# David-OConnor/molchanica

Hardware: AMD Instinct MI355X
Metric: MD atom-updates/sec (and steps/sec), 1M-atom solvated box (higher is better)
Workload: dtype f32

## Files before the change

molchanica_amd/csrc/mdx_api.hip:

```cpp
#include "mdx_comm.h"
#include <algorithm>
#include <atomic>
#include <chrono>
#include <cfloat>
#include <cmath>
#include <cstring>
#include <dlfcn.h>
#include <mutex>
#include <unordered_map>

static thread_local std::string g_last_error;
void mdx_set_error(const std::string& s) { g_last_error = s; }

static inline unsigned div_up(unsigned a, unsigned b) { return (a + b - 1) / b; }
static bool cut_on(float rc) { return rc > 0.f && std::isfinite(rc); }
static uint32_t f2u(float f) { uint32_t u; std::memcpy(&u, &f, 4); return u; }
static float u2f(uint32_t u) { float f; std::memcpy(&f, &u, 4); return f; }

#define FAIL(code, msg) do { mdx_set_error(msg); return (code); } while (0)

template <typename T>
static int upload_vec(T** dptr, const std::vector<T>& v, hipStream_t st) {
    if (*dptr) { (void)hipFree(*dptr); *dptr = nullptr; }
    HIP_TRY(hipMalloc((void**)dptr, std::max<size_t>(sizeof(T) * v.size(), 16)));
// ... 134 lines not shown
                    d.ps_cls, d.ps_p14, d.ps_stage, d.ps_slab, d.ps_rows, d.ps_fslab, d.ps_fout, d.ps_rigid, d.ps_flex, d.ps_flex_tab, d.ps_search, d.ps_cl, d.ps_cl_mat, d.gs_blk, d.gs_best, d.mx_blk};
    for (void* p : ptrs) if (p) (void)hipFree(p);
    d = DeviceState{};
}

extern "C" void mdx_destroy(mdx_handle* h) {
    if (!h) return;
    (void)hipSetDevice(h->device);
    if (h->stream) (void)hipStreamSynchronize(h->stream);
    mdx_dd_destroy(h);
    for (auto& e : h->ev_pending) { (void)hipEventDestroy(e.a); (void)hipEventDestroy(e.b); }
    for (auto& e : h->ev_pool) (void)hipEventDestroy(e);
    mdx_pme_destroy(h);
    free_device(h);
    if (h->h_ctl) (void)hipHostFree(h->h_ctl);
    if (h->h_rb) (void)hipHostFree(h->h_rb);
    if (h->stream) (void)hipStreamDestroy(h->stream);
    delete h;
}

static int create_impl(const mdx_system* s, const mdx_config* c, int device, mdx_handle* h) {
    const uint32_t N = s->n_atoms;
    h->N = N; h->cfg = *c; h->device = device;
    if (h->cfg.chunk_steps == 0) h->cfg.chunk_steps = N < 131072u ? 48u : 16u;
    if (h->cfg.chunk_steps > MDX_MAX_CHUNK) h->cfg.chunk_steps = MDX_MAX_CHUNK;
    decode_periodic(s->periodic, h->per);
    h->periodic = h->per[0] || h->per[1] || h->per[2];
    for (int d = 0; d < 3; ++d) h->posre_per[d] = h->per[d];
    for (int d = 0; d < 3; ++d) { h->box_lo[d] = s->box_lo[d]; h->box_hi[d] = s->box_hi[d]; }
    MDX_TRY(check_box(h->per, h->box_lo, h->box_hi, c));
    h->n_local = N; h->cap_local = N;
    const bool all_cut = cut_on(c->lj_cutoff) && cut_on(c->coulomb_cutoff);
    if (c->skin == 0.f && all_cut && h->periodic) {
        float s0 = 2.0f;
        for (int d = 0; d < 3; ++d)
            if (h->per[d]) s0 = std::min(s0, 0.5f * (h->box_hi[d] - h->box_lo[d]) - std::max(c->lj_cutoff, c->coulomb_cutoff) - 0.01f);
        if (s0 >= 0.5f) { h->cfg.skin = s0; h->skin_tune.on = true; h->skin_tune.base_skin = s0; MDX_TRY(check_box(h->per, h->box_lo, h->box_hi, &h->cfg)); }
    }
    h->r_list = all_cut ? std::max(c->lj_cutoff, c->coulomb_cutoff) + h->cfg.skin : INFINITY;

    int ndev = 0;
    if (hipGetDeviceCount(&ndev) != hipSuccess || ndev == 0) FAIL(MDX_EDEVICE, "no HIP device available");
    if (device < 0 || device >= ndev) FAIL(MDX_EDEVICE, "device index out of range");
    HIP_TRY(hipSetDevice(device));
    h->pme_cus_per_xcd = mdx_pme_cu_split(h, c);
    if (h->pme_cus_per_xcd) MDX_TRY(mdx_stream_create_masked(&h->stream, h->pme_cus_per_xcd, true));
    else HIP_TRY(hipStreamCreateWithFlags(&h->stream, hipStreamNonBlocking));
// ... 348 lines not shown
    if (h->profile_level == 2 && kind != 0 && kind != 4) return;
    if (h->profile_level == 2) {
        static const uint32_t every = [] { const char* e = std::getenv("MDX_PROF_SAMPLE"); const int v = e ? std::atoi(e) : 8; return (uint32_t)(v < 1 ? 1 : v); }();
        if (kind == 0) h->prof_sampled = (h->prof_seq++ % every) == 0u;
        if (!h->prof_sampled) return;
    }
    if (kind >= 6 && h->profile_level != 3) return;
    h->prof_open = true;
    mdx_handle::EvPair p{};
    p.kind = kind; p.tag = h->prof_tag; p.st = st ? st : h->stream;
    hipEvent_t* ev[2] = {&p.a, &p.b};
    for (auto e : ev) {
        if (!h->ev_pool.empty()) { *e = h->ev_pool.back(); h->ev_pool.pop_back(); }
        else (void)hipEventCreate(e);
    }
    (void)hipEventRecord(p.a, p.st);
    h->ev_pending.push_back(p);
}
void mdx_prof_end(mdx_handle* h) {
    if (!h->profile || !h->prof_open || h->ev_pending.empty()) return;
    h->prof_open = false;
    (void)hipEventRecord(h->ev_pending.back().b, h->ev_pending.back().st);
}
void mdx_prof_collect(mdx_handle* h, int first_stale_step) {
    for (auto& p : h->ev_pending) {
        float ms = 0.f;
        (void)hipEventSynchronize(p.b);
        const bool ran = p.tag < 0 || ((p.kind == 2 || p.kind == 5) ? p.tag <= first_stale_step : p.tag < first_stale_step);
        if (ran && hipEventElapsedTime(&ms, p.a, p.b) == hipSuccess) {
            if (p.kind == 0) { h->stats.nb_ms_sum += ms; h->stats.nb_launches++; }
            else if (p.kind == 4) h->stats.nb_ms_sum += ms;
            else if (p.kind == 1) { h->stats.bonded_ms_sum += ms; h->stats.bonded_launches++; }
            else if (p.kind == 2) { h->stats.integ_ms_sum += ms; h->stats.integ_launches++; }
            else if (p.kind == 5) { h->stats.fused_ms_sum += ms; h->stats.fused_launches++; }
            if (h->dd && h->profile_level == 3) {
                int ph = -1;
                if (p.kind >= 6 && p.kind <= 11) ph = p.kind - 6;
                else if (p.kind == 0) ph = MDX_PHASE_PAIR;
                else if (p.kind == 4) ph = MDX_PHASE_PAIR_BOUNDARY;
                else if (p.kind == 1 || p.kind == 5) ph = MDX_PHASE_BONDED;
                else if (p.kind == 2) ph = MDX_PHASE_INTEGRATE;
                if (ph >= 0) { h->dd->phase_ms[ph] += ms; h->dd->phase_n[ph]++; }
            }
        }
        h->ev_pool.push_back(p.a); h->ev_pool.push_back(p.b);
    }
    h->ev_pending.clear();
}

static void skin_apply(mdx_handle* h, float s) {
    h->cfg.skin = s;
    h->r_list = std::max(h->cfg.lj_cutoff, h->cfg.coulomb_cutoff) + s;
    h->list_valid = false;
    h->inner_skin_auto = 0.f; h->dual_auto_off = false; h->dual_win_steps = 0; h->dual_win_prunes = 0;
    h->stretch_samples = 0;
    h->skin_tune.win_steps = 0; h->skin_tune.win_rebuilds = 0; h->skin_tune.skip_rebuilds = 5;
}
static bool skin_fits(const mdx_handle* h, float s) {
    for (int d = 0; d < 3; ++d)
        if (h->per[d] && h->box_hi[d] - h->box_lo[d] < 2.0f * (std::max(h->cfg.lj_cutoff, h->cfg.coulomb_cutoff) + s)) return false;
    return true;
}
static void skin_autotune(mdx_handle* h, uint32_t done, bool stale_hit) {
    mdx_handle::SkinTune& t = h->skin_tune;
    const auto now = std::chrono::steady_clock::now();
    if (t.phase == 0) {
        t.warm_steps += done;
        if (t.warm_steps >= 200) { t.phase = 1; t.win_steps = 0; t.win_rebuilds = 0; t.skip_rebuilds = 1; }
        return;
    }
// ... 32 lines not shown
    const auto t0 = std::chrono::steady_clock::now();
    HIP_TRY(hipSetDevice(h->device));
    hipStream_t st = h->stream;
    DeviceState& d = h->d;
    const bool had_ext = h->have_ext;
    if (ext_forces) {
        if (h->n_local != h->N && !h->dd) FAIL(MDX_EPARAM, "external forces need the library's own decomposition (mdx_comm_init) on a narrowed handle");
        std::vector<float4> e4(h->N);
        for (uint32_t i = 0; i < h->N; ++i)
            e4[i] = make_float4(ext_forces[3 * i], ext_forces[3 * i + 1], ext_forces[3 * i + 2], 0.f);
        HIP_TRY(hipMemcpyAsync(d.ext_orig, e4.data(), sizeof(float4) * h->N, hipMemcpyHostToDevice, st));
        HIP_TRY(hipStreamSynchronize(st));
        h->have_ext = true; h->forces_valid = false;
    } else if (had_ext) {
        h->have_ext = false; h->forces_valid = false;
    }
    if (n_steps == 0) return MDX_OK;
    MDX_TRY(ensure_ready(h));
    if (h->moved_outside) { h->prune_pending = true; h->moved_outside = false; }
    uint32_t thr = stale_threshold_bits(h);
    uint32_t remaining = n_steps;
    while (remaining) {
        MDX_TRY(ensure_ready(h));
        uint32_t chunk = std::min(std::min(remaining, h->cfg.chunk_steps), mdx_steps_to_next_event(h));
        static const bool chunk_predict = [] { const char* e = std::getenv("MDX_CHUNK_PREDICT"); return !(e && e[0] == '0'); }();
        if (chunk_predict && h->stretch_samples >= 3 && chunk > 4) {
            const float left = h->stretch_mean + h->stretch_dev + 1.0f - (float)h->steps_since_rebuild;
            const uint32_t want = left > 4.0f ? (uint32_t)std::ceil(left) : 4u;
            chunk = std::min(chunk, want);
        }
        const auto t_chunk = std::chrono::steady_clock::now();
        MdxRange range_chunk("mdx step chunk");
        HIP_TRY(hipMemsetAsync(d.ctl, 0, sizeof(StepCtl), st));
        static const bool rattle_every = [] { const char* e = std::getenv("MDX_RATTLE_EVERY_STEP"); return e && e[0] == '1'; }();
        const int integ = h->integrator;
        const bool vv = integ == MDX_INTEGRATOR_VERLET_VELOCITY;
        const bool fused = vv && (!mdx_has_constraints(h) || !rattle_every);
        const bool fuse_bi = fused && mdx_bonded_integrate_ok(h);
        const bool want_e = mdx_energy_wanted_at(h, h->step_count + chunk);
        h->e_cache_valid = false; h->e_pending = false;
        const size_t e_bytes = sizeof(double) * (EN_COUNT + 8 + MDX_ESTRIDE * MDX_EPART);
        float4* pos_after[MDX_MAX_CHUNK + 1];
        const bool water = fused && mdx_water_step_ok(h);
        const bool pipe_chunk = fuse_bi && mdx_dd_fold_eligible(h);
        const bool onepass = fused && !water && !pipe_chunk && chunk >= (want_e ? 2u : 1u) && mdx_onepass_ok(h);
        float4* const ybuf[2] = {d.posq_alt, d.posq};
        float4* const fb3[3] = {d.force, d.force_b, d.force_c};
        auto onepass_point_at = [&](uint32_t n) {
// ... 71 lines not shown
        }
        h->prof_tag = -1;
        if (h->dd) { h->chunk_s = -1; mdx_dd_pipe_chunk_end(h); }
        static const bool dbg_host = [] { const char* e = std::getenv("MDX_DEBUG_HOST"); return e && e[0] == '1'; }();
        const auto t_enq = std::chrono::steady_clock::now();
        if (h->dd) h->dd->probe_both_buffers = fuse_bi && chunk > 1;
        MDX_TRY(ctl_to_host(h));
        if (h->dd) h->dd->probe_both_buffers = false;
        if (dbg_host && chunk >= 8) {
            static double enq = 0.0, wait = 0.0; static unsigned long long steps = 0, chunks = 0;
            const auto t_w = std::chrono::steady_clock::now();
            enq += std::chrono::duration<double, std::micro>(t_enq - t_chunk).count();
            wait += std::chrono::duration<double, std::micro>(t_w - t_enq).count();
            steps += chunk; ++chunks;
            if ((chunks & 31ull) == 0ull)
                std::fprintf(stderr, "[mdx host] %llu steps in %llu chunks: enqueue %.1f us per step, wait at the chunk end %.1f us per step\n",
                             steps, chunks, enq / (double)steps, wait / (double)steps);
        }
        uint32_t done = chunk;
        bool stale_hit = false;
        int first_stale = 1 << 30;
        for (uint32_t s = 0; s < chunk; ++s)
            if (h->h_ctl->disp2[s + 1] > thr || (onepass && h->h_ctl->viol[s])) { first_stale = (int)s; break; }
        if (h->profile) mdx_prof_collect(h, first_stale);
        static const bool dbg_stale = [] { const char* e = std::getenv("MDX_DEBUG_STALE"); return e && e[0] == '1'; }();
        if (dbg_stale && first_stale < (1 << 30))
            std::fprintf(stderr, "[mdx] list stale at step %d of a chunk of %u (step count %llu): word %.4g against (skin / 2)^2 = %.4g%s\n", first_stale, chunk,
                         (unsigned long long)h->step_count, (double)u2f(h->h_ctl->disp2[first_stale + 1]), (double)u2f(thr), h->dd ? " [decomposed]" : "");
        for (uint32_t s = 0; s < chunk; ++s) {
            const bool kick_beyond_grant = onepass && h->h_ctl->viol[s] != 0u;
            if (h->h_ctl->disp2[s + 1] > thr || kick_beyond_grant) {
                if (fuse_bi && !onepass && d.posq != pos_after[s]) std::swap(d.posq, d.posq_alt);
                if (onepass) {
                    onepass_point_at(s + 1);
                    MDX_TRY(mdx_launch_step_materialise(h, dt, ybuf[s & 1], fb3[s % 3], ybuf[(s + 1) & 1], kick_beyond_grant, s == 0 ? 0.5f : 1.0f, nullptr, 0));
                    if (kick_beyond_grant) ++h->onepass_violations;
                }
                if (u2f(h->h_ctl->disp2[s + 1]) > 1.0e29f) {
                    h->forces_valid = false; h->list_valid = false;
                    h->step_count += s;
                    FAIL(MDX_ENAN, "non-finite or runaway coordinates during mdx_step");
                }
                h->list_valid = false;
                const float len = (float)(h->steps_since_rebuild + s + 1);
                if (h->dd) { h->chunk_s = -1; MDX_TRY(mdx_dd_on_stale(h)); }
                else MDX_TRY(mdx_rebuild(h));
                {
                    if (h->stretch_samples == 0) { h->stretch_mean = len; h->stretch_dev = 2.0f; }
                    else {
                        h->stretch_dev += 0.25f * (std::fabs(len - h->stretch_mean) - h->stretch_dev);
                        h->stretch_mean += 0.25f * (len - h->stretch_mean);
                    }
                    ++h->stretch_samples;
                    stale_hit = true;
                }
                const bool e_now = want_e && s + 1 == chunk;
                if (e_now) HIP_TRY(hipMemsetAsync(d.energy, 0, e_bytes, st));
                h->nb_post_rebuild = !e_now;
                const int frc = compute_forces(h, e_now, nullptr, 0);
                h->nb_post_rebuild = false;
                MDX_TRY(frc);
                if (vv) {
                    MDX_TRY(mdx_launch_integrate(h, 2, dt, nullptr, nullptr, thr));
                    if (dt != 0.f) MDX_TRY(mdx_launch_constrain_velocities(h, nullptr, 0));
                }
                done = s + 1;
                break;
            }
        }
        if (h->dd) h->dd->spec_valid = false;
        if (h->dual_on && h->cfg.inner_skin == 0.f) {
            for (uint32_t s = 0; s < done; ++s) h->dual_win_prunes += h->h_ctl->prune[s + 1] != 0u;
            if (stale_hit && !h->inner_from_rebuild) ++h->dual_win_prunes;
            h->dual_win_steps += done;
            if (h->dual_win_steps >= 96) {
                const float f = (float)h->dual_win_prunes / (float)h->dual_win_steps;
                if (f > 0.30f) {
                    if (h->inner_skin + 0.25f <= h->cfg.skin - 0.75f) {
                        h->inner_skin_auto = h->inner_skin + 0.25f; h->inner_skin = h->inner_skin_auto;
                        h->prune_pending = true;
                    } else {
                        h->dual_auto_off = true; h->dual_on = false;
                    }
                }
                h->dual_win_steps = 0; h->dual_win_prunes = 0;
            }
        }
        if (h->dd && h->dd->world > 1 && h->dd->tune_phase < 2 && h->tile_split) {
            MdxDecomp* dd = h->dd;
            if (done == chunk && chunk == h->cfg.chunk_steps) {
                if (dd->tune_chunks >= 2) {
                    dd->tune_ms[dd->tune_phase] += std::chrono::duration<double, std::milli>(std::chrono::steady_clock::now() - t_chunk).count();
// ... 692 lines not shown
    if (n) hipLaunchKernelGGL(unpack_pos_kernel, dim3(div_up(n, 256)), dim3(256), 0, h->stream, n, d_gid,
                              h->d.slot_of, h->d.posq, (const float4*)d_in4, (const float4*)d_shift4,
                              flag_word >= 0 ? &h->d.ctl->disp2[flag_word] : nullptr,
                              dual ? h->d.ref : nullptr,
                              dual ? (mdx_dd_split_now(h) ? &h->d.ctl->prune_ghost[h->chunk_s + 1]
                                                                                                      : &h->d.ctl->prune[h->chunk_s + 1]) : nullptr,
                              0.5f * h->inner_skin * (1.0f - 1.0e-4f),
                              h->dd ? h->box_hi[0] - h->box_lo[0] : 0.f, h->dd ? h->box_hi[1] - h->box_lo[1] : 0.f,
                              h->dd ? h->box_hi[2] - h->box_lo[2] : 0.f, (dual && h->path_split) ? h->d.path : nullptr);
    HIP_TRY(hipGetLastError());
    h->forces_valid = false;
    if (!dual) h->moved_outside = true;
    return MDX_OK;
}

extern "C" void* mdx_stream(mdx_handle* h) { return h ? (void*)h->stream : nullptr; }
extern "C" int mdx_debug_half_stats(mdx_handle* h, unsigned long long out[6]) {
    HIP_TRY(hipStreamSynchronize(h->stream));
    HIP_TRY(hipMemcpy(out, h->d.inner_count + MDX_EPART, sizeof(unsigned long long) * 6, hipMemcpyDeviceToHost));
    return MDX_OK;
}

extern "C" int mdx_debug_pair_lists(mdx_handle* h, int which, uint32_t* dst, uint64_t capacity, uint64_t* n_out) {
    if (!h || !n_out || which < 0 || which > 5) FAIL(MDX_EPARAM, "bad argument");
    if (!h->in_slot_space || !h->d.list_counts || !h->d.entry_off) FAIL(MDX_EPARAM, "spatial caches not built");
    HIP_TRY(hipStreamSynchronize(h->stream));
    const DeviceState& d = h->d;
    const uint32_t T = h->T;
    const void* src = nullptr;
    uint64_t n = 0;
    if (which == 0) { src = d.list_counts; n = 2ull * T; }
    else if (which == 1) { src = d.entry_off; n = (uint64_t)T + 1; }
    else if (which == 4) { src = d.inner_nch; n = d.inner_nch ? 8ull * T : 0; }
    else if (which == 5) { src = d.orig_of; n = (uint64_t)T * MDX_TILE; }
    else {
        std::vector<ListCounts> cnt(T);
        std::vector<uint32_t> off((size_t)T + 1);
        if (T) HIP_TRY(hipMemcpy(cnt.data(), d.list_counts, sizeof(ListCounts) * T, hipMemcpyDeviceToHost));
        HIP_TRY(hipMemcpy(off.data(), d.entry_off, sizeof(uint32_t) * ((size_t)T + 1), hipMemcpyDeviceToHost));
        uint64_t ext = 0;
        for (uint32_t t = 0; t < T; ++t) ext = std::max<uint64_t>(ext, (uint64_t)off[t] + cnt[t].n_masked + cnt[t].n_plain);
        src = which == 2 ? d.entries : d.entries_in;
        n = src ? 2 * ext : 0;
    }
    *n_out = n;
    if (!dst) return MDX_OK;
    if (capacity < n) FAIL(MDX_EPARAM, "capacity below the number of words");
    if (n) HIP_TRY(hipMemcpy(dst, src, sizeof(uint32_t) * n, hipMemcpyDeviceToHost));
    return MDX_OK;
}

static int posre_install(mdx_handle* h) {
    DeviceState& d = h->d;
    hipStream_t st = h->stream;
    const uint32_t N = h->N, R_old = h->n_roles, n = h->n_posre;
    std::vector<uint32_t> off_old(N + 1);
    std::vector<RoleRec> rec_old(R_old);
// ... 104 lines not shown
```

molchanica_amd/csrc/mdx_grid.hip:

```cpp
#include "mdx_internal.h"
#include <atomic>
#include <chrono>
#include <algorithm>
#include <cfloat>
#include <cmath>

#define WAVE_LDS_SYNC()                                      \
    do {                                                     \
        __builtin_amdgcn_fence(__ATOMIC_SEQ_CST, "workgroup"); \
        __builtin_amdgcn_wave_barrier();                     \
    } while (0)

static inline unsigned div_up(unsigned a, unsigned b) { return (a + b - 1) / b; }

constexpr int SCAN_THREADS = 256;
constexpr int SCAN_ITEMS = 8;
constexpr int SCAN_TILE = SCAN_THREADS * SCAN_ITEMS;

template <int THREADS>
__device__ __forceinline__ uint32_t block_exclusive_scan(uint32_t v, uint32_t* s_wave , uint32_t* total) {
    const int lane = threadIdx.x & 63, wave = threadIdx.x >> 6;
    uint32_t inc = v;
#pragma unroll
    for (int d = 1; d < 64; d <<= 1) {
// ... 1290 lines not shown
    hipLaunchKernelGGL(readback_kernel, dim3(1), dim3(1), 0, h->stream, s, (volatile uint32_t*)h->h_rb, seq);
    if (h->profile) { HIP_TRY(hipStreamSynchronize(h->stream)); return MDX_OK; }
    return spin_on_readback(h, seq);
}

__global__ void cursor_sum_kernel(const unsigned long long* __restrict__ cursors, uint32_t* __restrict__ out) {
    const unsigned long long c = cursors[(size_t)threadIdx.x * 16];
    uint32_t e = (uint32_t)c, m = (uint32_t)(c >> 32);
#pragma unroll
    for (int k = 32; k > 0; k >>= 1) { e += __shfl_xor(e, k); m += __shfl_xor(m, k); }
    if (threadIdx.x == 0) { out[0] = e; out[1] = m; }
}

__global__ void pair_sum_kernel(unsigned long long* __restrict__ pc) {
    unsigned long long a = pc[(size_t)threadIdx.x * PC_STRIDE], b = pc[(size_t)threadIdx.x * PC_STRIDE + 1];
#pragma unroll
    for (int k = 32; k > 0; k >>= 1) { a += __shfl_xor(a, k); b += __shfl_xor(b, k); }
    if (threadIdx.x == 0) { pc[PC_TOTAL] = a; pc[PC_TOTAL + 1] = b; }
}

static float c_inner_skin(const mdx_config& c) { return c.inner_skin == 0.f ? 0.5f : c.inner_skin; }

constexpr uint32_t LPT_BUCKETS = 129;
enum { RB_T = 0, RB_T_OWN = 1, RB_NONFINITE = 2, RB_N_INT = 3, RB_SCAN_N = 4, RB_WORDS = 8 };

template <bool UNSORT>
__global__ __launch_bounds__(256) void rb_prep_kernel(uint32_t N, GridParams g, const uint32_t* __restrict__ gid, const uint32_t* __restrict__ slot_of,
                                                      const float4* __restrict__ posq, const float4* __restrict__ vel,
                                                      float4* __restrict__ pos_orig, float4* __restrict__ vel_orig,
                                                      const uint8_t* __restrict__ lflag, uint32_t* __restrict__ cell_of,
                                                      uint32_t* __restrict__ cell_k, uint32_t* __restrict__ cell_count,
                                                      uint32_t* __restrict__ nonfinite) {
    const uint32_t o = blockIdx.x * blockDim.x + threadIdx.x;
    if (o >= N) return;
    float4 p;
    if (UNSORT) { const uint32_t sl = slot_of[gid[o]]; p = posq[sl]; vel_orig[o] = vel[sl]; }
    else p = pos_orig[o];
    if (!(isfinite(p.x) && isfinite(p.y) && isfinite(p.z))) {
        *nonfinite = 1u;
        p.x = g.lo[0]; p.y = g.lo[1]; p.z = g.lo[2];
    }
    if (g.per[0]) p.x = wrap1(p.x, g.lo[0], g.len[0]);
    if (g.per[1]) p.y = wrap1(p.y, g.lo[1], g.len[1]);
    if (g.per[2]) p.z = wrap1(p.z, g.lo[2], g.len[2]);
    pos_orig[o] = p;
    const int cx = min(g.ncx - 1, max(0, mdx_col_of(g, 0, p.x)));
    const int cy = min(g.ncy - 1, max(0, mdx_col_of(g, 1, p.y)));
// ... 133 lines not shown
    }
    float lo[3] = {valid ? p.x : 3.0e38f, valid ? p.y : 3.0e38f, valid ? p.z : 3.0e38f};
    float hi[3] = {valid ? p.x : -3.0e38f, valid ? p.y : -3.0e38f, valid ? p.z : -3.0e38f};
#pragma unroll
    for (int m = 1; m < 8; m <<= 1)
#pragma unroll
        for (int d = 0; d < 3; ++d) { lo[d] = fminf(lo[d], __shfl_xor(lo[d], m)); hi[d] = fmaxf(hi[d], __shfl_xor(hi[d], m)); }
    const unsigned long long bv = __ballot(valid), bo = __ballot((fl & 2u) != 0);
    const unsigned long long kl = __ballot(l.y != 0.f), kq = __ballot(p.w != 0.f);
    if ((lane & 7) == 0) {
        const uint32_t c = t * MDX_CL_PER_TILE + (uint32_t)(lane >> 3);
        a.cl_lo[c] = make_float4(lo[0], lo[1], lo[2], (float)__popcll((bv >> lane) & 0xFFull));
        a.cl_hi[c] = make_float4(hi[0], hi[1], hi[2], (float)__popcll((bo >> lane) & 0xFFull));
        a.cl_kind[c] = (uint8_t)((((kl >> lane) & 0xFFull) ? 1u : 0u) | (((kq >> lane) & 0xFFull) ? 2u : 0u));
    }
}

struct LptSortLds { uint32_t hist[8 * LPT_BUCKETS], cur[8 * LPT_BUCKETS], scan[SCAN1_THREADS / 64]; };
__host__ __device__ inline uint32_t mdx_lpt_group_tiles(uint32_t T, uint32_t wpt) {
    const uint32_t tpb = (wpt > (uint32_t)MDX_NB_WAVES ? wpt : (uint32_t)MDX_NB_WAVES) / wpt;
    return (((T + tpb - 1u) / tpb + 7u) >> 3) * tpb;
}
__device__ __forceinline__ uint32_t lpt_counting_sort(uint32_t T, const ListCounts* __restrict__ counts, uint32_t group_tiles,
                                                      const uint32_t* __restrict__ is_int, uint32_t* __restrict__ order, LptSortLds& s) {
    constexpr uint32_t NB = 8 * LPT_BUCKETS;
    for (uint32_t b = threadIdx.x; b < NB; b += SCAN1_THREADS) s.hist[b] = 0;
    __syncthreads();
    auto bucket = [&](uint32_t t) {
        const uint32_t nch = (counts[t].n_masked + counts[t].n_plain) >> 3;
        const uint32_t major = group_tiles ? min(t / group_tiles, 7u) : ((is_int && !is_int[t]) ? 1u : 0u);
        return major * LPT_BUCKETS + LPT_BUCKETS - 1u - min(nch, LPT_BUCKETS - 1u);
    };
    for (uint32_t t = threadIdx.x; t < T; t += SCAN1_THREADS) atomicAdd(&s.hist[bucket(t)], 1u);
    __syncthreads();
    {
        const uint32_t b0 = 2u * threadIdx.x, h0 = b0 < NB ? s.hist[b0] : 0u, h1 = b0 + 1u < NB ? s.hist[b0 + 1u] : 0u;
        uint32_t tot;
        const uint32_t ex = block_exclusive_scan<SCAN1_THREADS>(h0 + h1, s.scan, &tot);
        if (b0 < NB) s.cur[b0] = ex;
        if (b0 + 1u < NB) s.cur[b0 + 1u] = ex + h0;
    }
    __syncthreads();
    const uint32_t n_major0 = s.cur[LPT_BUCKETS];
    __syncthreads();
    for (uint32_t t = threadIdx.x; t < T; t += SCAN1_THREADS) order[atomicAdd(&s.cur[bucket(t)], 1u)] = t;
    __syncthreads();
    return n_major0;
}

struct FinishArgs {
    uint32_t* rb_ctl; const ListCounts* counts;
    uint32_t* tile_lpt; uint32_t lpt_grouped; WptRule rule;
    const uint32_t* tile_int; uint32_t* tile_order;
    const unsigned long long* cursors; unsigned long long* pair_count; const uint32_t* flags;
    volatile uint32_t* host; uint32_t seq;
};
__global__ __launch_bounds__(SCAN1_THREADS) void rb_finish_kernel(FinishArgs a) {
    __shared__ LptSortLds s_sort;
    __shared__ uint32_t s_nint;
    const uint32_t T = a.rb_ctl[RB_T];
    if (threadIdx.x == 0) s_nint = 0u;
    if (a.tile_lpt) {
        const uint32_t group_tiles = a.lpt_grouped ? mdx_lpt_group_tiles(T, (uint32_t)mdx_wpt_rule(a.rule, T)) : 0u;
        (void)lpt_counting_sort(T, a.counts, group_tiles, nullptr, a.tile_lpt, s_sort);
    }
    if (a.tile_order) {
        const uint32_t n_int = lpt_counting_sort(T, a.counts, 0u, a.tile_int, a.tile_order, s_sort);
        if (threadIdx.x == 0) s_nint = n_int;
    }
    if (threadIdx.x < 64) {
        const unsigned long long c = a.cursors[(size_t)threadIdx.x * 16];
        uint32_t e = (uint32_t)c, m = (uint32_t)(c >> 32);
        unsigned long long pa = a.pair_count[(size_t)threadIdx.x * PC_STRIDE], pb = a.pair_count[(size_t)threadIdx.x * PC_STRIDE + 1];
#pragma unroll
        for (int k = 32; k > 0; k >>= 1) { e += __shfl_xor(e, k); m += __shfl_xor(m, k); pa += __shfl_xor(pa, k); pb += __shfl_xor(pb, k); }
        if (threadIdx.x == 0) {
            a.pair_count[PC_TOTAL] = pa; a.pair_count[PC_TOTAL + 1] = pb;
            a.rb_ctl[RB_N_INT] = s_nint;
            a.host[0] = T; a.host[1] = a.rb_ctl[RB_T_OWN]; a.host[2] = a.rb_ctl[RB_NONFINITE]; a.host[3] = s_nint;
            for (int k = 0; k < 4; ++k) a.host[4 + k] = a.flags[k];
            a.host[8] = e; a.host[9] = m;
            a.host[10] = (uint32_t)pa; a.host[11] = (uint32_t)(pa >> 32); a.host[12] = (uint32_t)pb; a.host[13] = (uint32_t)(pb >> 32);
            a.rb_ctl[RB_NONFINITE] = 0u;
            __threadfence_system();
            a.host[31] = a.seq;
        }
    }
}


struct RebuildKnobs {
    bool fused;
    bool two_pass;
    bool exact_prune;
    int inner_mode;
    uint32_t mw_below;
    bool list_debug;
    bool prune_hitbits;
    int prune_tries[2];
};
constexpr int PRUNE_HB_TRIES[2] = {1, 1};
constexpr uint32_t PRUNE_MW_BELOW_FUSED = 12000u, PRUNE_MW_BELOW_UNFUSED = 2048u;
static const RebuildKnobs& rebuild_knobs() {
    static const RebuildKnobs k = [] {
        auto env = [](const char* name) { const char* e = std::getenv(name); return e ? e : ""; };
        RebuildKnobs r;
        r.fused = env("MDX_REBUILD_FUSED")[0] != '0';
        r.two_pass = env("MDX_LIST_TWO_PASS")[0] == '1';
        r.exact_prune = env("MDX_EXACT_PRUNE")[0] != '0';
        const char in = env("MDX_REBUILD_INNER")[0];
        r.inner_mode = in == '0' ? 0 : (in == '2' ? 2 : 1);
        const char* const mw = std::getenv("MDX_PRUNE_MW_BELOW");
        r.mw_below = mw ? (uint32_t)std::atoi(mw) : PRUNE_MW_BELOW_FUSED;
        r.list_debug = std::getenv("MDX_LIST_DEBUG") != nullptr;
        r.prune_hitbits = env("MDX_PRUNE_HITBITS")[0] != '0';
        const char* const tr[2] = {std::getenv("MDX_PRUNE_TRIES"), std::getenv("MDX_PRUNE_TRIES_INNER")};
        for (int k = 0; k < 2; ++k) r.prune_tries[k] = tr[k] ? std::min(std::max(std::atoi(tr[k]), 0), 3) : PRUNE_HB_TRIES[k];
        return r;
    }();
    return k;
}

struct RebuildResult { uint32_t E = 0, MC = 0; unsigned long long npairs = 0; bool ordered = false, classified = false, inner_built = false; };

struct TileOrderPlan { bool lpt, grouped, split; };
static TileOrderPlan tile_order_plan(const mdx_handle* h, uint32_t T) {
    static const int lpt_env = [] { const char* e = std::getenv("MDX_TILE_LPT"); return e ? (e[0] == '0' ? 0 : (e[0] == '2' ? 2 : 1)) : -1; }();
    const bool decomposed = h->dd || h->n_local != h->N;
    TileOrderPlan p;
    p.lpt = (lpt_env >= 0 ? lpt_env >= 1 : (decomposed || T >= 512u)) && mdx_nb_variant(h) >= 2;
    p.grouped = lpt_env >= 0 ? lpt_env == 2 : !decomposed;
    p.split = h->want_tile_split && mdx_nb_variant(h) >= 2;
    return p;
}

static bool list_is_pruned(const mdx_handle* h) { return !std::isinf(h->r_list) && mdx_nb_variant(h) >= 2; }

static float next_inner_skin(const mdx_handle* h) { return h->inner_skin_auto > 0.f ? h->inner_skin_auto : c_inner_skin(h->cfg); }
static bool dual_list_wanted(const mdx_handle* h, float inner_skin) {
    return !h->dual_auto_off && mdx_nb_half(h) && list_is_pruned(h) && inner_skin > 0.f && inner_skin < h->cfg.skin &&
// ... 147 lines not shown
    ListArgs a = list_args(h, T_bound, d.rb_ctl + RB_T);
    launch_single_pass(h, &a);
    const bool inner_env = knobs.inner_mode == 2 || (knobs.inner_mode == 1 && !mdx_has_constraints(h) && h->n_vsites == 0);
    const float inner_skin_next = next_inner_skin(h);
    const bool inner_here = inner_env && prune && dual_list_wanted(h, inner_skin_next) && !h->dd && h->n_local == h->N && g.npop == 1 && !h->alch_on &&
                            d.entries_in && d.inner_nch;
    PruneInner pin{};
    if (inner_here) {
        pin.entries_in = d.entries_in; pin.inner_nch = d.inner_nch; pin.rule = mdx_wpt_rule_of(h);
        const float rin = std::max(std::isfinite(h->cfg.lj_cutoff) && h->cfg.lj_cutoff > 0.f ? h->cfg.lj_cutoff : 0.f,
                                   std::isfinite(h->cfg.coulomb_cutoff) && h->cfg.coulomb_cutoff > 0.f ? h->cfg.coulomb_cutoff : 0.f) + inner_skin_next;
        pin.rin2 = rin * rin;
    }
    const bool inner_launched = prune && launch_exact_prune(h, a, knobs.mw_below, d.rb_ctl, classify_here ? d.tile_bnd : nullptr, inner_here ? &pin : nullptr);
    MDX_TRY(mdx_remap_constraints(h));
    const uint32_t seq = ++h->rb_seq;
    {
        FinishArgs fa{};
        fa.rb_ctl = d.rb_ctl; fa.counts = d.list_counts;
        fa.tile_lpt = plan.lpt ? d.tile_lpt : nullptr; fa.lpt_grouped = plan.grouped ? 1u : 0u; fa.rule = mdx_wpt_rule_of(h);
        fa.tile_int = classify_here ? d.tile_bnd : nullptr; fa.tile_order = classify_here ? d.tile_order : nullptr;
        fa.cursors = reinterpret_cast<const unsigned long long*>(d.list_cursors); fa.pair_count = d.pair_count; fa.flags = d.flags_dev;
        fa.host = (volatile uint32_t*)h->h_rb; fa.seq = seq;
        hipLaunchKernelGGL(rb_finish_kernel, dim3(1), dim3(SCAN1_THREADS), 0, st, fa);
    }
    HIP_TRY(hipGetLastError());
    MDX_TRY(spin_on_readback(h, seq));
    const uint32_t T = h->h_rb[0], flags0 = h->h_rb[4];
    if (h->h_rb[2]) { h->cell_count_clean = false; mdx_set_error("non-finite position at neighbour rebuild"); return MDX_ENAN; }
    if (T > T_bound) { mdx_set_error("internal: tile count beyond its bound"); return MDX_EDEVICE; }
    h->T = T; h->S = (T + 1) * MDX_TILE;
    MDX_TRY(list_flags_error(flags0 & 1u));
    if (flags0 & (16u | 32u)) {
        if (knobs.list_debug) fprintf(stderr, "[mdx] fused list rebuild fell back: flags %u, T %u, cap_e %llu cap_m %u regions %u\n",
                                      flags0, T, (unsigned long long)h->cap_entries, h->cap_mchunks, a.n_regions);
        *fell_back = true;
        return MDX_OK;
    }
    MDX_TRY(list_flags_error(flags0));
    res->E = h->h_rb[8]; res->MC = h->h_rb[9];
    const unsigned long long built = (unsigned long long)h->h_rb[10] | ((unsigned long long)h->h_rb[11] << 32);
    const unsigned long long kept = (unsigned long long)h->h_rb[12] | ((unsigned long long)h->h_rb[13] << 32);
    res->npairs = prune ? kept : built;
    res->ordered = true;
    res->inner_built = inner_launched && mdx_wpt_rule(mdx_wpt_rule_of(h), T) == 1;
    h->force_zeroed = true;
    h->tile_lpt_on = plan.lpt; h->tile_lpt_grouped = plan.grouped;
// ... 155 lines not shown
        h->tile_split = false; h->n_interior = 0;
        if (plan.split) MDX_TRY(mdx_classify_tiles(h, plan.lpt));
    }
    if (!res.ordered) {
        h->tile_lpt_on = false;
        if (plan.lpt) MDX_TRY(mdx_order_tiles_by_length(h, plan.grouped));
    }
    h->list_valid = true;
    h->forces_valid = false;
    h->rebuild_count++; h->steps_since_rebuild = 0;
    mdx_dd_note_rebuild(h);
    h->inner_skin = next_inner_skin(h);
    h->dual_on = dual_list_wanted(h, h->inner_skin);
    h->prune_pending = !(res.inner_built && h->dual_on);
    h->inner_from_rebuild = !h->prune_pending;
    if (h->inner_from_rebuild) ++h->inner_rebuilds;
    h->tail_w = 0; h->tail_tiles = 0;
    if (h->dual_on && h->tile_lpt_on && h->tile_lpt_grouped && !h->alch_on) mdx_tail_plan(h, T, &h->tail_w, &h->tail_tiles);
    if (!d.inner_count) { ALLOC(d.inner_count, MDX_EPART + 8); HIP_TRY(hipMemsetAsync(d.inner_count, 0, sizeof(unsigned long long) * (MDX_EPART + 8), st)); }
    h->stats.n_atoms = h->n_local; h->stats.n_slots = S; h->stats.n_tiles = T; h->stats.n_clusters = NC;
    h->stats.n_list_entries = res.E; h->stats.n_masked_entries = (uint64_t)res.MC * 8;
    h->stats.n_cluster_pairs = (mdx_nb_variant(h) >= 2) ? res.npairs : (uint64_t)res.E * 8;
    if (h->profile) {
        float ms = 0.f;
        HIP_TRY(hipEventRecord(e1, st)); HIP_TRY(hipEventSynchronize(e1));
        HIP_TRY(hipEventElapsedTime(&ms, e0, e1));
        h->stats.rebuild_ms_sum += ms;
        h->ev_pool.push_back(e0); h->ev_pool.push_back(e1);
    }
    return MDX_OK;
}

__global__ __launch_bounds__(SCAN1_THREADS) void lpt_order_kernel(uint32_t T, const ListCounts* __restrict__ counts, const uint32_t* __restrict__ is_int,
                                                                  uint32_t* __restrict__ order, uint32_t group_tiles) {
    __shared__ LptSortLds s_sort;
    (void)lpt_counting_sort(T, counts, group_tiles, is_int, order, s_sort);
}

__global__ __launch_bounds__(256) void tile_class_kernel(uint32_t T, const uint8_t* __restrict__ slot_flags,
                                                         const ListCounts* __restrict__ counts, const uint32_t* __restrict__ entry_off,
                                                         const uint2* __restrict__ entries, uint32_t* __restrict__ tile_bnd) {
    const uint32_t t = blockIdx.x * 4 + (threadIdx.x >> 6);
    const int lane = threadIdx.x & 63;
    if (t >= T) return;
    const uint8_t f = slot_flags[t * MDX_TILE + lane];
    bool ghost = (f & 1u) && !(f & 2u);
    const ListCounts c = counts[t];
    const uint32_t e0 = entry_off[t], n = c.n_masked + c.n_plain;
    for (uint32_t k = lane; k < n; k += 64) {
        const uint2 e = entries[e0 + k];
        if (((e.y >> 8) & 0xFFu) == 0u) continue;
// ... 106 lines not shown
```

molchanica_amd/csrc/mdx_internal.h:

```cpp
#pragma once
#include <hip/hip_runtime.h>
#include <stdint.h>
#include <chrono>
#include <cstdlib>
#include <cstring>
#include <string>
#include <vector>
#include "../../include/mdx.h"

#define MDX_TILE 64
#define MDX_CLUSTER 8
#define MDX_CL_PER_TILE 8
#define MDX_ACC_CONV 418.4f
#define MDX_KB 0.0019872041
#define MDX_INVALID 0xFFFFFFFFu
#define MDX_DUMMY_BASE 1.0e6f
#define MDX_DUMMY_STEP 64.0f
#define MDX_MAX_CHUNK 64
#define MDX_MAX_GROUPS 255

#define MDX_ESTRIDE 5
#define MDX_EPART 256
enum { EN_BOND = 0, EN_ANGLE, EN_DIHEDRAL, EN_LJ, EN_COUL, EN_LJ14, EN_COUL14, EN_KIN, EN_RECIP, EN_VIRIAL, EN_POSRE, EN_POSRE_VIR, EN_COUNT };

// ... 263 lines not shown
    bool dual_on = false;
    float inner_skin = 0.f;
    float inner_skin_auto = 0.f; bool dual_auto_off = false; uint32_t dual_win_steps = 0, dual_win_prunes = 0;
    bool prune_pending = true;
    uint32_t inner_rebuilds = 0;
    bool inner_from_rebuild = false;
    bool path_split = false;
    OnePassNow onepass;
    bool onepass_refused = false;
    uint64_t onepass_launches = 0, onepass_violations = 0;
    bool prune_latch = false;
    bool moved_outside = true;
    void (*wait_hook)(void*) = nullptr; void* wait_hook_arg = nullptr;
    bool kind_split = false;
    uint32_t n_interior = 0;
    bool tile_split = false;
    bool tile_lpt_on = false;
    bool tile_lpt_grouped = false;
    bool want_tile_split = false; uint32_t cap_tile_split = 0;
    int nb_step = -1;
    uint32_t energy_every = 0; bool e_pending = false, e_cache_valid = false; uint64_t e_cache_step = 0; mdx_energies e_cache{};
    bool nb_post_rebuild = false;
    uint32_t steps_since_rebuild = 0, stretch_samples = 0; float stretch_mean = 0.f, stretch_dev = 0.f;
    struct SkinTune {
        bool on = false; int phase = 0;
        float base_skin = 2.f, best_skin = 2.f, trial = 2.f; double base_rate = 0.0, best_rate = 0.0;
        uint32_t win_steps = 0, win_rebuilds = 0, skip_rebuilds = 0, warm_steps = 0;
        float dt_tuned = 0.f;
        std::chrono::steady_clock::time_point t0;
    } skin_tune;
    int chunk_s = -1;
    bool list_valid = false;
    bool forces_valid = false;
    bool in_slot_space = false;
    bool have_ext = false;
    uint64_t step_count = 0, rebuild_count = 0;
    bool profile = false; int profile_level = 0; bool prof_open = false;
    struct EvPair { hipEvent_t a, b; int kind; int tag; hipStream_t st; };
    int prof_tag = -1;
    uint32_t prof_seq = 0; bool prof_sampled = false;
    std::vector<EvPair> ev_pending;
    std::vector<hipEvent_t> ev_pool;
    mdx_stats stats{};
    int tstat_kind = 0; float tstat_temp = 300.f, tstat_tau = 1.f; uint32_t tstat_every = 10;
    int integrator = 0; float lang_gamma = 1.f, lang_temp = 300.f; uint64_t lang_seed = 0, lang_step = 0;
    int baro_kind = 0; float baro_p0 = 1.f, baro_tau = 5.f, baro_beta = 4.5e-5f; uint32_t baro_every = 25;
// ... 198 lines not shown
int mdx_groups_evaluate(mdx_handle* h, float* out );
bool mdx_mixing_on(const mdx_handle* h);
int mdx_mixing_evaluate(mdx_handle* h, mdx_solubility* out, double* atom_sums_or_null);
int mdx_foreign_evaluate(mdx_handle* h, double* du );
int mdx_launch_scale_velocities(mdx_handle* h, float lambda, const double* com_v_or_null);
int mdx_launch_momentum(mdx_handle* h);

static inline bool mdx_has_constraints(const mdx_handle* h) { return h->n_groups != 0 || h->n_star5 != 0; }
static inline double mdx_dof(const mdx_handle* h) {
    const double d = 3.0 * (double)h->n_mobile - (double)h->n_cons - 3.0;
    return d < 1.0 ? 1.0 : d;
}

#include "mdx_splitmix64.h"

void mdx_range_push(const char* name);
void mdx_range_pop();
struct MdxRange {
    explicit MdxRange(const char* name) { mdx_range_push(name); }
    ~MdxRange() { mdx_range_pop(); }
    MdxRange(const MdxRange&) = delete; MdxRange& operator=(const MdxRange&) = delete;
};

void mdx_prof_begin(mdx_handle* h, int kind, hipStream_t st = nullptr);
void mdx_prof_end(mdx_handle* h);
void mdx_prof_collect(mdx_handle* h, int first_stale_step = 1 << 30);
```

molchanica_amd/md_state.py:

```python
from __future__ import annotations

import ctypes as C
import os

import numpy as np

from ._abi import (CCommDiag, CFlexOpts, CGuestFlex, CGuestLigand, CHBond, CConfig, CEnergies, CLUSTER_MAX_PERMS, CLUSTER_MAX_POSES, CLUSTER_POSES_ARGTYPES, CRefineOpts,
                   CSearchOpts, CStats, CSystem, FLEX_DIHEDRALS, FORCE, FUSED_TRIAD_INFO_ARGTYPES, POSE_RMSD_ARGTYPES,
                   MDX_EDEVICE, MDX_ENAN, MDX_EOOM, MDX_EPARAM, MDX_OK, POS, POSE_MAX_ATOMS, POSE_MAX_TORSIONS, GUEST_FORCES_ARGTYPES, REFINE_GUESTS_ARGTYPES, REFINE_GUESTS_FLEX_ARGTYPES, SCREEN_LIGANDS_ARGTYPES, VEL, GuestFlex, GuestLigand,
                   MdConfig, MdSystem, CSolubility, SET_SOLUTE_COPIES_ARGTYPES, SNAPSHOT_READ_SOLUBILITY_ARGTYPES, SOLUBILITY_MIXING_ARGTYPES,
                   SOLUTE_MAX_COPIES)

_HERE = os.path.dirname(os.path.abspath(__file__))
LIB_PATH = os.environ.get("MDX_LIB") or os.path.join(_HERE, "libmdx.so")


class ParamError(ValueError):
    """The reference's `ParamError { descrip }` (src/md/mod.rs:967)."""


class DeviceError(RuntimeError):
    """HIP/device failure (MDX_EDEVICE / MDX_EOOM); the reference degrades to its CPU path here
    (src/util.rs:1072-1119) — this library has none and says so loudly."""

# ... 666 lines not shown
        _check(load_library().mdx_upload(self._h, VEL, a.ctypes.data_as(_fp)))

    def set_cell(self, lo, hi):
        _check(load_library().mdx_set_box(self._h, (C.c_float * 3)(*map(float, lo)),
                                          (C.c_float * 3)(*map(float, hi))))

    def shrink_cell_towards(self, target_lo, target_hi, shrink_per_step: float) -> bool:
        lo = (C.c_float * 3)(*[float(v) for v in target_lo]); hi = (C.c_float * 3)(*[float(v) for v in target_hi])
        out = C.c_int(0)
        _check(load_library().mdx_shrink_cell_towards(self._h, lo, hi, float(shrink_per_step), C.byref(out)))
        return bool(out.value)

    def rebuild_spatial_caches(self):
        _check(load_library().mdx_rebuild_spatial_caches(self._h))

    def neighbor_list(self):
        lib = load_library()
        off = np.zeros(self.n_atoms + 1, dtype=np.uint32)
        _check(lib.mdx_neighbor_list(self._h, off.ctypes.data_as(_u32p), None))
        idx = np.zeros(max(int(off[-1]), 1), dtype=np.uint32)
        _check(lib.mdx_neighbor_list(self._h, off.ctypes.data_as(_u32p), idx.ctypes.data_as(_u32p)))
        return off, idx[: int(off[-1])]

    PAIR_LIST_ARRAYS = ("counts", "entry_off", "entries", "entries_in", "inner_nch", "orig_of")

    def debug_pair_lists(self):
        lib = load_library()
        out = {}
        for which, name in enumerate(self.PAIR_LIST_ARRAYS):
            n = C.c_uint64(0)
            _check(lib.mdx_debug_pair_lists(self._h, which, None, 0, C.byref(n)))
            a = np.zeros(int(n.value), dtype=np.uint32)
            if a.size:
                _check(lib.mdx_debug_pair_lists(self._h, which, a.ctypes.data_as(_u32p), a.size, C.byref(n)))
            out[name] = a
        for name, w in (("counts", 2), ("entries", 2), ("entries_in", 2), ("inner_nch", 8), ("orig_of", 64)):
            out[name] = out[name].reshape(-1, w)
        return out

    def minimize_energy(self, max_iters: int, external_forces=None, f_tol: float = 0.0):
        ext = None
        if external_forces is not None:
            ext = np.ascontiguousarray(external_forces, dtype=np.float32).reshape(self.n_atoms, 3)
        e, it = CEnergies(), C.c_uint32(0)
        _check(load_library().mdx_minimize_energy(self._h, int(max_iters), None if ext is None else ext.ctypes.data_as(_fp),
                                                  float(f_tol), C.byref(e), C.byref(it)))
        return e.as_dict(), int(it.value)
# ... 360 lines not shown
```

Baseline: 2.307 billion.

## Lengthen predicted chunks, split LPT sort across blocks, defer rebuild timing sync

For large systems, once the stretch predictor has at least three samples, the step-chunk cap rises from 16 to 32 (capped further by the predicted steps until the next rebuild), cutting host round-trips. The rebuild finish kernel now runs the grouped LPT counting sort across 8 blocks, each sorting its own tile group, and the last block to finish does the rest. Rebuild profiling events are queued for deferred collection instead of a blocking event sync, and profile collection is delayed when a chunk goes stale. Longer chunks risk wasted speculative steps when the list goes stale mid-chunk, and the multi-block finish adds an atomic completion counter.

```diff
diff --git a/molchanica_amd/csrc/mdx_api.hip b/molchanica_amd/csrc/mdx_api.hip
--- a/molchanica_amd/csrc/mdx_api.hip
+++ b/molchanica_amd/csrc/mdx_api.hip
@@ -180,7 +180,9 @@
 static int create_impl(const mdx_system* s, const mdx_config* c, int device, mdx_handle* h) {
     const uint32_t N = s->n_atoms;
     h->N = N; h->cfg = *c; h->device = device;
-    if (h->cfg.chunk_steps == 0) h->cfg.chunk_steps = N < 131072u ? 48u : 16u;
+    static const bool cap_all = [] { const char* e = std::getenv("MDX_CHUNK_CAP_ALL"); return e && e[0] == '1'; }();
+    h->chunk_long = h->cfg.chunk_steps == 0 && (N >= 131072u || cap_all);
+    if (h->cfg.chunk_steps == 0) h->cfg.chunk_steps = h->chunk_long ? 16u : 48u;
     if (h->cfg.chunk_steps > MDX_MAX_CHUNK) h->cfg.chunk_steps = MDX_MAX_CHUNK;
     decode_periodic(s->periodic, h->per);
     h->periodic = h->per[0] || h->per[1] || h->per[2];
@@ -575,8 +577,10 @@
     h->prof_open = false;
     (void)hipEventRecord(h->ev_pending.back().b, h->ev_pending.back().st);
 }
-void mdx_prof_collect(mdx_handle* h, int first_stale_step) {
-    for (auto& p : h->ev_pending) {
+void mdx_prof_collect(mdx_handle* h, int first_stale_step, size_t n_first) {
+    n_first = std::min(n_first, h->ev_pending.size());
+    for (size_t k = 0; k < n_first; ++k) {
+        auto& p = h->ev_pending[k];
         float ms = 0.f;
         (void)hipEventSynchronize(p.b);
         const bool ran = p.tag < 0 || ((p.kind == 2 || p.kind == 5) ? p.tag <= first_stale_step : p.tag < first_stale_step);
@@ -586,6 +590,7 @@
             else if (p.kind == 1) { h->stats.bonded_ms_sum += ms; h->stats.bonded_launches++; }
             else if (p.kind == 2) { h->stats.integ_ms_sum += ms; h->stats.integ_launches++; }
             else if (p.kind == 5) { h->stats.fused_ms_sum += ms; h->stats.fused_launches++; }
+            else if (p.kind == MDX_PROF_KIND_REBUILD) h->stats.rebuild_ms_sum += ms;
             if (h->dd && h->profile_level == 3) {
                 int ph = -1;
                 if (p.kind >= 6 && p.kind <= 11) ph = p.kind - 6;
@@ -598,7 +603,7 @@
         }
         h->ev_pool.push_back(p.a); h->ev_pool.push_back(p.b);
     }
-    h->ev_pending.clear();
+    h->ev_pending.erase(h->ev_pending.begin(), h->ev_pending.begin() + (std::ptrdiff_t)n_first);
 }
 
 static void skin_apply(mdx_handle* h, float s) {
@@ -677,8 +682,10 @@
     uint32_t remaining = n_steps;
     while (remaining) {
         MDX_TRY(ensure_ready(h));
-        uint32_t chunk = std::min(std::min(remaining, h->cfg.chunk_steps), mdx_steps_to_next_event(h));
         static const bool chunk_predict = [] { const char* e = std::getenv("MDX_CHUNK_PREDICT"); return !(e && e[0] == '0'); }();
+        static const uint32_t chunk_cap = [] { const char* e = std::getenv("MDX_CHUNK_CAP"); return e ? (uint32_t)std::min(std::max(std::atoi(e), 0), MDX_MAX_CHUNK) : 32u; }();
+        const bool long_now = h->chunk_long && !h->dd && chunk_predict && h->stretch_samples >= 3;
+        uint32_t chunk = std::min(std::min(remaining, long_now ? std::max(chunk_cap, h->cfg.chunk_steps) : h->cfg.chunk_steps), mdx_steps_to_next_event(h));
         if (chunk_predict && h->stretch_samples >= 3 && chunk > 4) {
             const float left = h->stretch_mean + h->stretch_dev + 1.0f - (float)h->steps_since_rebuild;
             const uint32_t want = left > 4.0f ? (uint32_t)std::ceil(left) : 4u;
@@ -796,7 +803,10 @@
         int first_stale = 1 << 30;
         for (uint32_t s = 0; s < chunk; ++s)
             if (h->h_ctl->disp2[s + 1] > thr || (onepass && h->h_ctl->viol[s])) { first_stale = (int)s; break; }
-        if (h->profile) mdx_prof_collect(h, first_stale);
+        static const bool collect_early = [] { const char* e = std::getenv("MDX_PROF_COLLECT_EARLY"); return e && e[0] == '1'; }();
+        const size_t n_ev_chunk = h->ev_pending.size();
+        const bool collect_late = h->profile && !collect_early && !h->dd && first_stale < (1 << 30);
+        if (h->profile && !collect_late) mdx_prof_collect(h, first_stale);
         static const bool dbg_stale = [] { const char* e = std::getenv("MDX_DEBUG_STALE"); return e && e[0] == '1'; }();
         if (dbg_stale && first_stale < (1 << 30))
             std::fprintf(stderr, "[mdx] list stale at step %d of a chunk of %u (step count %llu): word %.4g against (skin / 2)^2 = %.4g%s\n", first_stale, chunk,
@@ -813,6 +823,7 @@
                 if (u2f(h->h_ctl->disp2[s + 1]) > 1.0e29f) {
                     h->forces_valid = false; h->list_valid = false;
                     h->step_count += s;
+                    if (collect_late) mdx_prof_collect(h, first_stale, n_ev_chunk);
                     FAIL(MDX_ENAN, "non-finite or runaway coordinates during mdx_step");
                 }
                 h->list_valid = false;
@@ -842,6 +853,7 @@
                 break;
             }
         }
+        if (collect_late) mdx_prof_collect(h, first_stale, n_ev_chunk);
         if (h->dd) h->dd->spec_valid = false;
         if (h->dual_on && h->cfg.inner_skin == 0.f) {
             for (uint32_t s = 0; s < done; ++s) h->dual_win_prunes += h->h_ctl->prune[s + 1] != 0u;
@@ -1580,7 +1592,7 @@
 }
 
 extern "C" int mdx_debug_pair_lists(mdx_handle* h, int which, uint32_t* dst, uint64_t capacity, uint64_t* n_out) {
-    if (!h || !n_out || which < 0 || which > 5) FAIL(MDX_EPARAM, "bad argument");
+    if (!h || !n_out || which < 0 || which > 6) FAIL(MDX_EPARAM, "bad argument");
     if (!h->in_slot_space || !h->d.list_counts || !h->d.entry_off) FAIL(MDX_EPARAM, "spatial caches not built");
     HIP_TRY(hipStreamSynchronize(h->stream));
     const DeviceState& d = h->d;
@@ -1591,6 +1603,7 @@
     else if (which == 1) { src = d.entry_off; n = (uint64_t)T + 1; }
     else if (which == 4) { src = d.inner_nch; n = d.inner_nch ? 8ull * T : 0; }
     else if (which == 5) { src = d.orig_of; n = (uint64_t)T * MDX_TILE; }
+    else if (which == 6) { src = d.tile_lpt; n = (h->tile_lpt_on && d.tile_lpt) ? T : 0; }
     else {
         std::vector<ListCounts> cnt(T);
         std::vector<uint32_t> off((size_t)T + 1);
diff --git a/molchanica_amd/csrc/mdx_grid.hip b/molchanica_amd/csrc/mdx_grid.hip
--- a/molchanica_amd/csrc/mdx_grid.hip
+++ b/molchanica_amd/csrc/mdx_grid.hip
@@ -1336,7 +1336,7 @@
 static float c_inner_skin(const mdx_config& c) { return c.inner_skin == 0.f ? 0.5f : c.inner_skin; }
 
 constexpr uint32_t LPT_BUCKETS = 129;
-enum { RB_T = 0, RB_T_OWN = 1, RB_NONFINITE = 2, RB_N_INT = 3, RB_SCAN_N = 4, RB_WORDS = 8 };
+enum { RB_T = 0, RB_T_OWN = 1, RB_NONFINITE = 2, RB_N_INT = 3, RB_SCAN_N = 4, RB_FINISH_DONE = 5, RB_WORDS = 8 };
 
 template <bool UNSORT>
 __global__ __launch_bounds__(256) void rb_prep_kernel(uint32_t N, GridParams g, const uint32_t* __restrict__ gid, const uint32_t* __restrict__ slot_of,
@@ -1516,8 +1516,10 @@
     return (((T + tpb - 1u) / tpb + 7u) >> 3) * tpb;
 }
 __device__ __forceinline__ uint32_t lpt_counting_sort(uint32_t T, const ListCounts* __restrict__ counts, uint32_t group_tiles,
-                                                      const uint32_t* __restrict__ is_int, uint32_t* __restrict__ order, LptSortLds& s) {
+                                                      const uint32_t* __restrict__ is_int, uint32_t* __restrict__ order, LptSortLds& s,
+                                                      uint32_t t_lo = 0u, uint32_t t_hi = 0xFFFFFFFFu) {
     constexpr uint32_t NB = 8 * LPT_BUCKETS;
+    t_hi = min(t_hi, T);
     for (uint32_t b = threadIdx.x; b < NB; b += SCAN1_THREADS) s.hist[b] = 0;
     __syncthreads();
     auto bucket = [&](uint32_t t) {
@@ -1525,7 +1527,7 @@
         const uint32_t major = group_tiles ? min(t / group_tiles, 7u) : ((is_int && !is_int[t]) ? 1u : 0u);
         return major * LPT_BUCKETS + LPT_BUCKETS - 1u - min(nch, LPT_BUCKETS - 1u);
     };
-    for (uint32_t t = threadIdx.x; t < T; t += SCAN1_THREADS) atomicAdd(&s.hist[bucket(t)], 1u);
+    for (uint32_t t = t_lo + threadIdx.x; t < t_hi; t += SCAN1_THREADS) atomicAdd(&s.hist[bucket(t)], 1u);
     __syncthreads();
     {
         const uint32_t b0 = 2u * threadIdx.x, h0 = b0 < NB ? s.hist[b0] : 0u, h1 = b0 + 1u < NB ? s.hist[b0 + 1u] : 0u;
@@ -1537,7 +1539,7 @@
     __syncthreads();
     const uint32_t n_major0 = s.cur[LPT_BUCKETS];
     __syncthreads();
-    for (uint32_t t = threadIdx.x; t < T; t += SCAN1_THREADS) order[atomicAdd(&s.cur[bucket(t)], 1u)] = t;
+    for (uint32_t t = t_lo + threadIdx.x; t < t_hi; t += SCAN1_THREADS) order[t_lo + atomicAdd(&s.cur[bucket(t)], 1u)] = t;
     __syncthreads();
     return n_major0;
 }
@@ -1552,11 +1554,27 @@
 __global__ __launch_bounds__(SCAN1_THREADS) void rb_finish_kernel(FinishArgs a) {
     __shared__ LptSortLds s_sort;
     __shared__ uint32_t s_nint;
+    __shared__ uint32_t s_last;
     const uint32_t T = a.rb_ctl[RB_T];
     if (threadIdx.x == 0) s_nint = 0u;
     if (a.tile_lpt) {
         const uint32_t group_tiles = a.lpt_grouped ? mdx_lpt_group_tiles(T, (uint32_t)mdx_wpt_rule(a.rule, T)) : 0u;
-        (void)lpt_counting_sort(T, a.counts, group_tiles, nullptr, a.tile_lpt, s_sort);
+        if (gridDim.x > 1u) {
+            const uint32_t lo = blockIdx.x * group_tiles;
+            if (lo < T) (void)lpt_counting_sort(T, a.counts, group_tiles, nullptr, a.tile_lpt, s_sort, lo, blockIdx.x + 1u == gridDim.x ? T : lo + group_tiles);
+        } else {
+            (void)lpt_counting_sort(T, a.counts, group_tiles, nullptr, a.tile_lpt, s_sort);
+        }
+    }
+    if (gridDim.x > 1u) {
+        __syncthreads();
+        if (threadIdx.x == 0) {
+            __threadfence();
+            s_last = atomicAdd(&a.rb_ctl[RB_FINISH_DONE], 1u) + 1u == gridDim.x ? 1u : 0u;
+        }
+        __syncthreads();
+        if (!s_last) return;
+        if (threadIdx.x == 0) a.rb_ctl[RB_FINISH_DONE] = 0u;
     }
     if (a.tile_order) {
         const uint32_t n_int = lpt_counting_sort(T, a.counts, 0u, a.tile_int, a.tile_order, s_sort);
@@ -1592,6 +1610,8 @@
     bool list_debug;
     bool prune_hitbits;
     int prune_tries[2];
+    bool finish_split;
+    bool timer_sync;
 };
 constexpr int PRUNE_HB_TRIES[2] = {1, 1};
 constexpr uint32_t PRUNE_MW_BELOW_FUSED = 12000u, PRUNE_MW_BELOW_UNFUSED = 2048u;
@@ -1610,6 +1630,8 @@
         r.prune_hitbits = env("MDX_PRUNE_HITBITS")[0] != '0';
         const char* const tr[2] = {std::getenv("MDX_PRUNE_TRIES"), std::getenv("MDX_PRUNE_TRIES_INNER")};
         for (int k = 0; k < 2; ++k) r.prune_tries[k] = tr[k] ? std::min(std::max(std::atoi(tr[k]), 0), 3) : PRUNE_HB_TRIES[k];
+        r.timer_sync = env("MDX_REBUILD_TIMER_SYNC")[0] == '1';
+        r.finish_split = env("MDX_FINISH_SPLIT")[0] != '0';
         return r;
     }();
     return k;
@@ -1803,7 +1825,8 @@
         fa.tile_int = classify_here ? d.tile_bnd : nullptr; fa.tile_order = classify_here ? d.tile_order : nullptr;
         fa.cursors = reinterpret_cast<const unsigned long long*>(d.list_cursors); fa.pair_count = d.pair_count; fa.flags = d.flags_dev;
         fa.host = (volatile uint32_t*)h->h_rb; fa.seq = seq;
-        hipLaunchKernelGGL(rb_finish_kernel, dim3(1), dim3(SCAN1_THREADS), 0, st, fa);
+        const bool split8 = knobs.finish_split && fa.tile_lpt && plan.grouped && !fa.tile_order;
+        hipLaunchKernelGGL(rb_finish_kernel, dim3(split8 ? 8 : 1), dim3(SCAN1_THREADS), 0, st, fa);
     }
     HIP_TRY(hipGetLastError());
     MDX_TRY(spin_on_readback(h, seq));
@@ -2005,11 +2028,16 @@
     h->stats.n_list_entries = res.E; h->stats.n_masked_entries = (uint64_t)res.MC * 8;
     h->stats.n_cluster_pairs = (mdx_nb_variant(h) >= 2) ? res.npairs : (uint64_t)res.E * 8;
     if (h->profile) {
-        float ms = 0.f;
-        HIP_TRY(hipEventRecord(e1, st)); HIP_TRY(hipEventSynchronize(e1));
-        HIP_TRY(hipEventElapsedTime(&ms, e0, e1));
-        h->stats.rebuild_ms_sum += ms;
-        h->ev_pool.push_back(e0); h->ev_pool.push_back(e1);
+        HIP_TRY(hipEventRecord(e1, st));
+        if (knobs.timer_sync) {
+            float ms = 0.f;
+            HIP_TRY(hipEventSynchronize(e1));
+            HIP_TRY(hipEventElapsedTime(&ms, e0, e1));
+            h->stats.rebuild_ms_sum += ms;
+            h->ev_pool.push_back(e0); h->ev_pool.push_back(e1);
+        } else {
+            h->ev_pending.push_back(mdx_handle::EvPair{e0, e1, MDX_PROF_KIND_REBUILD, -1, st});
+        }
     }
     return MDX_OK;
 }
diff --git a/molchanica_amd/csrc/mdx_internal.h b/molchanica_amd/csrc/mdx_internal.h
--- a/molchanica_amd/csrc/mdx_internal.h
+++ b/molchanica_amd/csrc/mdx_internal.h
@@ -309,6 +309,7 @@
     uint32_t energy_every = 0; bool e_pending = false, e_cache_valid = false; uint64_t e_cache_step = 0; mdx_energies e_cache{};
     bool nb_post_rebuild = false;
     uint32_t steps_since_rebuild = 0, stretch_samples = 0; float stretch_mean = 0.f, stretch_dev = 0.f;
+    bool chunk_long = false;
     struct SkinTune {
         bool on = false; int phase = 0;
         float base_skin = 2.f, best_skin = 2.f, trial = 2.f; double base_rate = 0.0, best_rate = 0.0;
@@ -553,6 +554,7 @@
     MdxRange(const MdxRange&) = delete; MdxRange& operator=(const MdxRange&) = delete;
 };
 
+#define MDX_PROF_KIND_REBUILD 12
 void mdx_prof_begin(mdx_handle* h, int kind, hipStream_t st = nullptr);
 void mdx_prof_end(mdx_handle* h);
-void mdx_prof_collect(mdx_handle* h, int first_stale_step = 1 << 30);
+void mdx_prof_collect(mdx_handle* h, int first_stale_step = 1 << 30, size_t n_first = ~(size_t)0);
diff --git a/molchanica_amd/md_state.py b/molchanica_amd/md_state.py
--- a/molchanica_amd/md_state.py
+++ b/molchanica_amd/md_state.py
@@ -712,7 +712,7 @@
         _check(lib.mdx_neighbor_list(self._h, off.ctypes.data_as(_u32p), idx.ctypes.data_as(_u32p)))
         return off, idx[: int(off[-1])]
 
-    PAIR_LIST_ARRAYS = ("counts", "entry_off", "entries", "entries_in", "inner_nch", "orig_of")
+    PAIR_LIST_ARRAYS = ("counts", "entry_off", "entries", "entries_in", "inner_nch", "orig_of", "tile_lpt")
 
     def debug_pair_lists(self):
         lib = load_library()
```

After: 2.321 billion (median of 6 runs). No clear change (+0.6%).
